# luciddreamer-cvlab/LucidDreamer

Hardware: AMD Instinct MI355X
Metric: views/sec fwd+bwd @1080p (1e6 Gaussians) (higher is better)
Workload: dtype f32

## Files before the change

### luciddreamer_amd/csrc/api.hip

```cpp
#include "common.h"
#include "../../include/lucid_raster.h"
#include "lr_src_hash.h"

#include <cstdio>
#include <cstdlib>
#include <cstddef>
#include <cstring>
#include <cmath>
#include <map>
#include <atomic>
#include <chrono>
#include <mutex>
#include <thread>
#include <string>
#include <vector>

namespace {

thread_local std::string g_last_error;

int fail(int code, const std::string& msg)
{
    g_last_error = msg;
    return code;
// ... 215 lines not shown
        return a.buf;
    }
    if (a.P != P) return nullptr;
    for (int k = 0; k < 5; k++) if (a.tgt[k] != tgt[k]) return nullptr;
    return a.buf;
}

struct RawArgs { const float* sh_rest; const float* opacity_raw; float* dL_dsh_rest; };

static int forward_core(lr_alloc_fn geom_alloc, void* geom_user, lr_alloc_fn binning_alloc, void* binning_user,
               lr_alloc_fn img_alloc, void* img_user, int P, int D, int M, const float* background,
               int width, int height, const float* means3D, const float* shs, const float* colors_precomp,
               const float* opacities, const float* scales, float scale_modifier, const float* rotations,
               const float* cov3D_precomp, const float* viewmatrix, const float* projmatrix,
               const float* cam_pos, float tan_fovx, float tan_fovy, int prefiltered, float* out_color,
               float* out_depth, int* radii, int debug, long long binning_capacity, void* stream_, const RawArgs* raw)
{
    using namespace lr;
    const bool antialiasing = g_antialiasing.load(std::memory_order_relaxed) != 0;
    hipStream_t s = reinterpret_cast<hipStream_t>(stream_);
    const bool early_header = g_early_request;
    g_early_request = false;
    const bool reset_sticky = take_reset_sticky();
    if (P < 0 || width <= 0 || height <= 0) return fail(LR_ERR_INVALID_ARG, "P, width, height must be positive");
    if (!geom_alloc || !binning_alloc || !img_alloc) return fail(LR_ERR_INVALID_ARG, "allocator callbacks are required");
    if (!background || !viewmatrix || !projmatrix || !cam_pos || !out_color || !out_depth)
        return fail(LR_ERR_INVALID_ARG, "background/viewmatrix/projmatrix/cam_pos/out_color/out_depth are required");
    if (P > 0 && (!means3D || !opacities || !radii)) return fail(LR_ERR_INVALID_ARG, "means3D/opacities/radii are required");
    if (P > 0 && shs == nullptr && colors_precomp == nullptr)
        return fail(LR_ERR_INVALID_ARG, "For non-RGB, provide precomputed Gaussian colors!");
    if (P > 0 && cov3D_precomp == nullptr && (scales == nullptr || rotations == nullptr))
        return fail(LR_ERR_INVALID_ARG, "provide scales+rotations or cov3D_precomp");
    if (shs != nullptr && (D < 0 || D > 3 || (D + 1) * (D + 1) > M))
        return fail(LR_ERR_INVALID_ARG, "SH degree must be 0..3 and (D+1)^2 <= M");
    if (binning_capacity < 0 || binning_capacity > 0xFFFFFFF0ll) return fail(LR_ERR_INVALID_ARG, "bad binning_capacity");

    const int gx = (width + TILE_X - 1) / TILE_X, gy = (height + TILE_Y - 1) / TILE_Y;
    const int num_tiles = gx * gy;

    const GeomLayout GL = geom_layout(P);
    const ImgLayout IL = img_layout(width, height);
// ... 110 lines not shown
                                               R_bound, &bp, scratch->words, (uint32_t)n_sum_words, s);
            if (rc == -2) return fail(LR_ERR_INVALID_ARG, "image / instance count too large: tile and slot bits exceed the 64-bit sort word");
            if (rc != 0) return fail(LR_ERR_HIP, "could not reserve LDS for the binning kernels");
            ranges_written = true;
            guard.armed = false;
            LR_DEBUG_SYNC(debug, s, "tile binning");
        }
    } else {
        (void)binning_alloc(bin_layout(0).total, binning_user);
    }
    if (!ranges_written) LR_HIP_CHECK(hipMemsetAsync(ranges, 0, (size_t)num_tiles * sizeof(uint2), s));

    { ProfScope ps(ST_RENDER_FWD, s);
    launch_render_fwd(width, height, gx, gy, ranges, point_list, list_gid, rec, background, final_T, n_contrib, out_color,
                      out_depth, quad_hits, hdr, seg_list, ckpt, reinterpret_cast<uint32_t*>(img + IL.tile_seg0),
                      reinterpret_cast<float4*>(img + IL.c_final), inst_hint, s); }
    LR_DEBUG_SYNC(debug, s, "render");
    LR_HIP_CHECK(hipGetLastError());

    if (binning_capacity == 0 && prefiltered && P > 0) {
        uint32_t trap = 0;
        LR_HIP_CHECK(hipMemcpyAsync(&trap, &hdr->prefilter_trap, 4, hipMemcpyDeviceToHost, s));
        LR_HIP_CHECK(hipStreamSynchronize(s));
        if (trap) return fail(LR_ERR_PREFILTERED, "Point is filtered although prefiltered is set. This shouldn't happen!");
    }
    return num_rendered;
}

int lr_forward(lr_alloc_fn geom_alloc, void* geom_user, lr_alloc_fn binning_alloc, void* binning_user,
               lr_alloc_fn img_alloc, void* img_user, int P, int D, int M, const float* background,
               int width, int height, const float* means3D, const float* shs, const float* colors_precomp,
// ... 403 lines not shown
    unsigned int mask = LR_ACC_MEAN2D | LR_ACC_OPACITY | LR_ACC_MEAN3D;
    if (a->acc_color) mask |= LR_ACC_COLOR;
    if (a->acc_cov3D) mask |= LR_ACC_COV3D;
    if (a->acc_sh) mask |= LR_ACC_SH;
    if (a->acc_scale) mask |= LR_ACC_SCALE;
    if (a->acc_rot) mask |= LR_ACC_ROT;

    lr::ViewsInFlight overlap(n_streams);
    for (int v = 0; v < n_views; v++) {
        const int si = v % n_streams;
        hipStream_t s = g_view_streams[si];
        char* slot = workspace + (size_t)si * SL.total;
        SliceCookie cg = { slot + SL.geom, SL.img - SL.geom }, ci = { slot + SL.img, SL.bin - SL.img },
                    cb = { slot + SL.bin, SL.color - SL.bin };
        float* color = (a->out_color && a->out_color[v]) ? a->out_color[v] : reinterpret_cast<float*>(slot + SL.color);
        float* depth = (a->out_depth && a->out_depth[v]) ? a->out_depth[v] : reinterpret_cast<float*>(slot + SL.depth);
        int* radii = (a->out_radii && a->out_radii[v]) ? a->out_radii[v] : reinterpret_cast<int*>(slot + SL.radii);
        g_reset_sticky = v < n_streams;
        int rc = lr_forward(slice_alloc, &cg, slice_alloc, &cb, slice_alloc, &ci, P, D, M, a->background, width, height,
                            a->means3D, a->shs, a->colors_precomp, a->opacities, a->scales, a->scale_modifier, a->rotations,
                            a->cov3D_precomp, a->viewmatrices[v], a->projmatrices[v], a->cam_positions[v], a->tan_fovx[v],
                            a->tan_fovy[v], 0, color, depth, radii, 0, binning_capacity, s);
        if (rc < 0 && rc != LR_NUM_RENDERED_ON_DEVICE) return rc;
        const float* view_grad = with_loss ? nullptr : a->dL_dpix[v];
        const float* view_depth_grad = a->dL_ddepth ? a->dL_ddepth[v] : nullptr;
        const float* view_alpha_grad = a->dL_dalpha ? a->dL_dalpha[v] : nullptr;
        float* alpha_out = (a->out_alpha && a->out_alpha[v]) ? a->out_alpha[v] : nullptr;
        const float* final_T = reinterpret_cast<const float*>(slot + SL.img + img_layout(width, height).final_T);
        if (alpha_out && !with_mask_loss) launch_render_alpha(final_T, (long long)width * height, alpha_out, s);
        if (with_loss) {
            const float* cmask = with_mask_loss ? masks[v] : nullptr;
            float* gimg = reinterpret_cast<float*>(slot + SL.grad_img);
            float* out_v = a->out_losses + loss_stride * (size_t)v;
            launch_loss_forward(3, height, width, color, targets[v], a->lambda_dssim, out_v, slot + SL.loss_ws, s, true, cmask);
            launch_loss_backward(3, height, width, color, targets[v], a->lambda_dssim, nullptr, slot + SL.loss_ws, gimg, s, out_v,
                                 nullptr, cmask);
            view_grad = gimg;
// ... 597 lines not shown
```

### luciddreamer_amd/csrc/common.h

```cpp
#pragma once
#include <hip/hip_runtime.h>
#include <stdint.h>
#include <stddef.h>

namespace lr {

constexpr int TILE_X = 16;
constexpr int TILE_Y = 16;
constexpr int TILE_PIX = TILE_X * TILE_Y;
constexpr int WAVE = 64;

struct __attribute__((aligned(16))) GaussRec {
    float x, y, ca, cb;
    float cc, opacity, r, g;
    float b, depth, qmax, pad1;
};
static_assert(sizeof(GaussRec) == 48, "GaussRec must be 48 bytes");

struct __attribute__((aligned(16))) GradRec {
    float dmx, dmy, dca, dcb;
    float dcc, dop, dr, dg;
    float db, pad0, pad1, pad2;
};
static_assert(sizeof(GradRec) == 48, "GradRec must be 48 bytes");
// ... 281 lines not shown
enum { TILE_MAP_BANDS = 0, TILE_MAP_PLAIN = 1 };
int blend_tile_map(int num_tiles);
__device__ __forceinline__ int blend_tile(int map, int num_tiles)
{
    int t = (int)blockIdx.x;
    if (map == TILE_MAP_BANDS) {
        const int per = (num_tiles + 7) >> 3;
        t = (int)(blockIdx.x & 7) * per + (int)(blockIdx.x >> 3);
    }
    return t < num_tiles ? t : -1;
}
void launch_render_fwd(int W, int H, int gx, int gy, const uint2* ranges, const uint32_t* point_list,
                       const uint32_t* list_gid, const GaussRec* rec, const float* bg, float* final_T,
                       uint32_t* n_contrib, float* out_color, float* out_depth, uint8_t* quad_hits,
                       GeomHeader* hdr, uint2* seg_list, float4* ckpt, uint32_t* tile_seg0, float4* c_final,
                       long long inst_hint, hipStream_t s);
void launch_render_alpha(const float* final_T, long long n, float* alpha, hipStream_t s);
void launch_render_bwd(int W, int H, int gx, int gy, const uint2* ranges, const uint32_t* point_list,
                       const GaussRec* rec, const float* bg, const float* final_T,
                       const uint32_t* n_contrib, const float* dL_dpix, char* bin_base, const GeomHeader* hdr,
                       const uint32_t* tile_seg0, const float4* c_final, long long seg_bound, hipStream_t s,
                       const float* dL_ddepth = nullptr, const float* depth_img = nullptr, const float* dL_dalpha = nullptr);
__device__ __forceinline__ void adam_one(float gi, float& mi, float& vi, float& pi, float w1, float beta2, float w2,
                                         float bc2_sqrt, float eps, float step_size)
{
    mi = __builtin_fmaf(w1, gi - mi, mi);
    vi = vi * beta2;
    vi = __builtin_fmaf(w2 * gi, gi, vi);
    const float denom = sqrtf(vi) / bc2_sqrt + eps;
    pi = __builtin_fmaf(-step_size, mi / denom, pi);
}
// ... 57 lines not shown
```

### luciddreamer_amd/csrc/preprocess.hip

```cpp
#include <cstddef>
#include "common.h"

namespace lr {

namespace {

__device__ constexpr float SH_C0 = 0.28209479177387814f;
__device__ constexpr float SH_C1 = 0.4886025119029199f;
__device__ constexpr float SH_C2[5] = { 1.0925484305920792f, -1.0925484305920792f, 0.31539156525252005f,
                                        -1.0925484305920792f, 0.5462742152960396f };
__device__ constexpr float SH_C3[7] = { -0.5900435899266435f, 2.890611442640554f, -0.4570457994644658f,
                                        0.3731763325901154f, -0.4570457994644658f, 1.445305721320277f,
                                        -0.5900435899266435f };

struct M3 { float c[3][3]; };

__device__ __forceinline__ M3 m3_mul(const M3& A, const M3& B)
{
    M3 R;
#pragma unroll
    for (int j = 0; j < 3; j++)
#pragma unroll
        for (int i = 0; i < 3; i++)
            R.c[j][i] = A.c[0][i] * B.c[j][0] + A.c[1][i] * B.c[j][1] + A.c[2][i] * B.c[j][2];
// ... 83 lines not shown
    res.x += 0.5f; res.y += 0.5f; res.z += 0.5f;
    clamp_bits = (uint8_t)((res.x < 0 ? 1 : 0) | (res.y < 0 ? 2 : 0) | (res.z < 0 ? 4 : 0));
    res.x = fmaxf(res.x, 0.0f); res.y = fmaxf(res.y, 0.0f); res.z = fmaxf(res.z, 0.0f);
    return res;
}

__device__ __forceinline__ void tile_rect(float px, float py, int radius, int gx, int gy,
                                          int& minx, int& miny, int& maxx, int& maxy)
{
    minx = min(gx, max(0, (int)((px - radius) / TILE_X)));
    miny = min(gy, max(0, (int)((py - radius) / TILE_Y)));
    maxx = min(gx, max(0, (int)((px + radius + TILE_X - 1) / TILE_X)));
    maxy = min(gy, max(0, (int)((py + radius + TILE_Y - 1) / TILE_Y)));
}

constexpr int PP_THREADS = 128;
constexpr int PP_WAVES = PP_THREADS / 64;

template <bool RAW, bool AA>
__global__ void __launch_bounds__(PP_THREADS)
k_preprocess(ViewParams vp, const float* __restrict__ means3D, const float* __restrict__ scales,
             const float* __restrict__ rotations, const float* __restrict__ opacities,
             const float* __restrict__ shs, const float* __restrict__ cov3D_precomp,
             const float* __restrict__ colors_precomp, int prefiltered,
             int* __restrict__ radii, GaussRec* __restrict__ rec, uint8_t* __restrict__ clamped,
             uint32_t* __restrict__ tiles_touched, uint4* __restrict__ hitrec,
             uint32_t* __restrict__ depth_key, GeomHeader* hdr, uint32_t binning_capacity,
             uint32_t* __restrict__ chunk_sums)
{
    __shared__ uint32_t s_list[PP_THREADS];
    __shared__ uint32_t s_wcnt[PP_WAVES];
    const int gid = blockIdx.x * blockDim.x + threadIdx.x;
    uint32_t* const trap = chunk_sums != nullptr ? chunk_sums + 4 * ((size_t)(vp.P + SCAN_TILE - 1) / SCAN_TILE) : &hdr->prefilter_trap;
    const float* __restrict__ V = vp.view;
    const float* __restrict__ Pm = vp.proj;
    {
        const bool in_range = gid < vp.P;
        const size_t li = in_range ? (size_t)gid : 0;
        const float vz1 = V[2] * means3D[3 * li] + V[6] * means3D[3 * li + 1] + V[10] * means3D[3 * li + 2] + V[14];
        const bool pass = in_range && !(vz1 <= 0.2f);
        if (in_range && !pass) {
            if (prefiltered) *trap = 1;
            radii[gid] = 0; tiles_touched[gid] = 0;
            if (depth_key) depth_key[gid] = 0xFFFFFFFFu;
        }
        const uint64_t m = __ballot(pass);
        const int w = threadIdx.x >> 6, l = threadIdx.x & 63;
// ... 12 lines not shown
    const int idx = live ? (int)s_list[threadIdx.x] : 0;

    int radius_out = 0;
    uint32_t tiles_out = 0;
    uint32_t area_ref = 0;
    uint32_t key_out = 0xFFFFFFFFu;

    const size_t li = (size_t)idx;
    const float px_w = means3D[3 * li], py_w = means3D[3 * li + 1], pz_w = means3D[3 * li + 2];
    const float vx = V[0] * px_w + V[4] * py_w + V[8] * pz_w + V[12];
    const float vy = V[1] * px_w + V[5] * py_w + V[9] * pz_w + V[13];
    const float vz = V[2] * px_w + V[6] * py_w + V[10] * pz_w + V[14];

    do {
        if (!live) break;
        const float hx = Pm[0] * px_w + Pm[4] * py_w + Pm[8] * pz_w + Pm[12];
        const float hy = Pm[1] * px_w + Pm[5] * py_w + Pm[9] * pz_w + Pm[13];
        const float hw = Pm[3] * px_w + Pm[7] * py_w + Pm[11] * pz_w + Pm[15];
        const float p_w = 1.0f / (hw + 0.0000001f);
        const float ndcx = hx * p_w, ndcy = hy * p_w;

        float c3[6];
        if (cov3D_precomp != nullptr) {
#pragma unroll
            for (int i = 0; i < 6; i++) c3[i] = cov3D_precomp[6 * (size_t)idx + i];
        } else {
            float sx = scales[3 * (size_t)idx], sy = scales[3 * (size_t)idx + 1], sz = scales[3 * (size_t)idx + 2];
            const float4 q = reinterpret_cast<const float4*>(rotations)[idx];
            float r = q.x, x = q.y, y = q.z, z = q.w;
            if (RAW) {
// ... 236 lines not shown
    __shared__ uint16_t s_near[PL_POOL];
    __shared__ int s_radius[PL_POOL];
    __shared__ uint32_t s_tiles[PL_POOL];
    __shared__ float s_mid[6][PL_POOL];
    __shared__ float s_coef[AA ? PL_POOL : 1];
    __shared__ uint32_t s_mid_id[PL_POOL];
    __shared__ uint32_t s_tests[PL_POOL];
    __shared__ uint2 s_rect[PL_POOL];
    __shared__ uint32_t s_mask[PL_POOL][2];
    __shared__ uint32_t s_wcnt[PL_ROUNDS * PL_WAVES];
    __shared__ uint32_t s_nmid;
    __shared__ uint32_t s_sum[3];
    const int tid = threadIdx.x, w = tid >> 6, l = tid & 63;
    const int base = blockIdx.x * PL_POOL;
    uint32_t* const trap = chunk_sums != nullptr ? chunk_sums + 4 * ((size_t)(vp.P + SCAN_TILE - 1) / SCAN_TILE) : &hdr->prefilter_trap;
    if (tid == 0) { s_nmid = 0u; s_sum[0] = 0u; s_sum[1] = 0u; s_sum[2] = 0u; }
    const float* __restrict__ V = vp.view;

    bool pass[PL_ROUNDS];
    uint64_t m[PL_ROUNDS];
#pragma unroll
    for (int r = 0; r < PL_ROUNDS; r++) {
        const int loc = r * PL_THREADS + tid, gid = base + loc;
        const bool in_range = gid < vp.P;
        const size_t li = in_range ? (size_t)gid : 0;
        const float vz1 = V[2] * means3D[3 * li] + V[6] * means3D[3 * li + 1] + V[10] * means3D[3 * li + 2] + V[14];
        pass[r] = in_range && !(vz1 <= 0.2f);
        if (in_range && !pass[r] && prefiltered) *trap = 1;
        s_radius[loc] = 0; s_tiles[loc] = 0u;
        m[r] = __ballot(pass[r]);
        if (l == 0) s_wcnt[r * PL_WAVES + w] = (uint32_t)__popcll(m[r]);
    }
    lds_barrier();
    uint32_t n_near = 0;
#pragma unroll
    for (int r = 0; r < PL_ROUNDS; r++) {
        uint32_t before = n_near;
#pragma unroll
        for (int i = 0; i < PL_WAVES; i++) { if (i < w) before += s_wcnt[r * PL_WAVES + i]; n_near += s_wcnt[r * PL_WAVES + i]; }
        if (pass[r]) s_near[before + __popcll(m[r] & ((1ull << l) - 1ull))] = (uint16_t)(r * PL_THREADS + tid);
    }
    lds_barrier();

    for (uint32_t i0 = 0; i0 < n_near; i0 += PL_THREADS) {
        const uint32_t i = i0 + (uint32_t)tid;
        Projected pj;
        bool ok = false;
        uint32_t loc = 0;
        if (i < n_near) {
            loc = s_near[i];
            ok = project_gaussian<RAW, AA>(vp, base + (int)loc, means3D, scales, rotations, cov3D_precomp, pj);
        }
        const uint64_t mk = __ballot(ok);
        uint32_t wbase = 0;
        if (l == 0 && mk != 0ull) wbase = atomicAdd(&s_nmid, (uint32_t)__popcll(mk));
        wbase = (uint32_t)__shfl((int)wbase, 0);
        if (ok) {
            const uint32_t slot = wbase + (uint32_t)__popcll(mk & ((1ull << l) - 1ull));
            s_mid[0][slot] = pj.pix; s_mid[1][slot] = pj.piy; s_mid[2][slot] = pj.con_a; s_mid[3][slot] = pj.con_b;
            s_mid[4][slot] = pj.con_c; s_mid[5][slot] = pj.vz;
            if constexpr (AA) s_coef[slot] = pj.coef;
            s_mid_id[slot] = loc; s_radius[loc] = pj.radius;
        }
    }
    lds_barrier();
// ... 151 lines not shown
```

### luciddreamer_amd/csrc/render_fwd.hip

```cpp
#include "common.h"

namespace lr {

namespace {

constexpr int THREADS = 256;
constexpr int NWAVES = THREADS / 64;
constexpr int BATCH = 256;

struct PixState { float T, Cr, Cg, Cb, D, acc; uint32_t last; };

template <bool STRICT>
__device__ __forceinline__ void fwd_pixel(PixState& p, uint64_t& done, const float qA, const float qB, const float qC,
                                          const float r0, const float r1,
                                          const float dx, const float op, const float cr, const float cg, const float cb,
                                          const float depth, const uint32_t pos0)
{
    float power;
    const float alpha = fminf(0.99f, op * gauss_weight<STRICT>(qA, qB, qC, r0, r1, dx, power));
    const float test_T = p.T * (1.0f - alpha);
    const uint64_t pass = ~done & __builtin_amdgcn_ballot_w64(power <= 0.0f) & __builtin_amdgcn_ballot_w64(alpha >= 1.0f / 255.0f);
    const uint64_t low_T = __builtin_amdgcn_ballot_w64(test_T < 0.0001f);
    const uint64_t stop = pass & low_T;
    const bool use = __builtin_amdgcn_inverse_ballot_w64(pass & ~low_T);
    done |= stop;
    const float wgt = use ? alpha * p.T : 0.f;
    p.Cr += cr * wgt; p.Cg += cg * wgt; p.Cb += cb * wgt; p.D += depth * wgt; p.acc += wgt;
    p.T = use ? test_T : p.T;
    if (stop != 0ull) {
        asm volatile("");
        p.last = __builtin_amdgcn_inverse_ballot_w64(stop) ? pos0 : p.last;
    }
}

__device__ __forceinline__ void fwd_step(PixState& p, uint64_t& done, const float alpha, const float power, const uint64_t enable,
                                         const float cr, const float cg, const float cb, const float depth, const uint32_t pos0)
{
    const float test_T = p.T * (1.0f - alpha);
    const uint64_t pass = enable & ~done & __builtin_amdgcn_ballot_w64(power <= 0.0f) & __builtin_amdgcn_ballot_w64(alpha >= 1.0f / 255.0f);
    const uint64_t low_T = __builtin_amdgcn_ballot_w64(test_T < 0.0001f);
    const uint64_t stop = pass & low_T;
    const bool use = __builtin_amdgcn_inverse_ballot_w64(pass & ~low_T);
    done |= stop;
    const float wgt = use ? alpha * p.T : 0.f;
    p.Cr += cr * wgt; p.Cg += cg * wgt; p.Cb += cb * wgt; p.D += depth * wgt; p.acc += wgt;
    p.T = use ? test_T : p.T;
    p.last = __builtin_amdgcn_inverse_ballot_w64(stop) ? pos0 : p.last;
}

constexpr int PAIR_MIN_LIST = 1024;
template <bool STRICT, bool PAIR>
__global__ void __launch_bounds__(THREADS)
k_render_fwd(int W, int H, int gx, int num_tiles, int tile_map, const uint2* __restrict__ ranges,
             const uint32_t* __restrict__ point_list, const uint32_t* __restrict__ list_gid,
             const GaussRec* __restrict__ rec,
             const float* __restrict__ bg, float* __restrict__ final_T, uint32_t* __restrict__ n_contrib,
             float* __restrict__ out_color, float* __restrict__ out_depth, uint8_t* __restrict__ quad_hits,
             GeomHeader* __restrict__ hdr, uint2* __restrict__ seg_list, float4* __restrict__ ckpt,
             uint32_t* __restrict__ tile_seg0, float4* __restrict__ c_final)
{
    __shared__ float4 s_q0[BATCH];
    __shared__ float4 s_q1[BATCH];
    __shared__ float4 s_q2[BATCH];
    __shared__ float2 s_q3[BATCH];
    __shared__ int s_wdone[NWAVES];
    __shared__ uint32_t s_seg0;

    const int tile = blend_tile(tile_map, num_tiles);
    if (tile < 0) return;
    const int tx = tile % gx, ty = tile / gx;
    const int tid = threadIdx.x, w = tid >> 6, l = tid & 63;
    const int x0 = tx * TILE_X + (w & 1) * 8, y0 = ty * TILE_Y + (w >> 1) * 8;
    const int px = x0 + (l & 7), py = y0 + (l >> 3);
    const bool inside = px < W && py < H;
    const float pxf = (float)px, pyf = (float)py;
    const float bx0 = (float)x0, bx1 = (float)(x0 + 7), by0 = (float)y0, by1 = (float)(y0 + 7);

    const uint2 range = ranges[tile];
    const int total = (int)(range.y - range.x);

    PixState A = { 1.0f, 0.f, 0.f, 0.f, 0.f, 0.000001f, 0u };
    uint64_t done = __builtin_amdgcn_ballot_w64(!inside);
    bool wave_done = done == ~0ull;

    static_assert(BATCH == BWD_SEG, "a staging round of the forward is one segment of the backward");
    const int n_seg = total > 0 ? (total - 1) / BWD_SEG : 0;
    uint32_t seg0 = 0;
    int n_ck = 0;
    if (n_seg > 0) {
        if (tid == 0) { s_seg0 = atomicAdd(&hdr->n_seg, (uint32_t)n_seg); tile_seg0[tile] = s_seg0; }
        lds_barrier();
        seg0 = s_seg0;
        for (int g = 1 + tid; g <= n_seg; g += THREADS) seg_list[seg0 + g - 1] = make_uint2((uint32_t)tile, (uint32_t)g);
    }

    for (int base = 0; base < total; base += BATCH) {
// ... 37 lines not shown
                    mask &= mask - 1;
                    const bool two = mask != 0ull;
                    const int k1 = two ? __ffsll((long long)mask) - 1 : k0;
                    mask &= mask - 1;
                    const int j0 = sb + k0, j1 = sb + k1;
                    float4 a0 = s_q0[j0], a1 = s_q0[j1];
                    float4 b0 = s_q1[j0], b1 = s_q1[j1];
                    const float4 c0 = s_q2[j0], c1 = s_q2[j1];
                    asm volatile("" : "+v"(a0.x), "+v"(a0.y), "+v"(a0.z), "+v"(a0.w), "+v"(b0.x), "+v"(a1.x), "+v"(a1.y), "+v"(a1.z), "+v"(a1.w), "+v"(b1.x));
                    float r00, r01, r10, r11, power0, power1;
                    gauss_row<STRICT>(a0.w, b0.x, a0.y - pyf, r00, r01);
                    gauss_row<STRICT>(a1.w, b1.x, a1.y - pyf, r10, r11);
                    float alpha0 = fminf(0.99f, b0.y * gauss_weight<STRICT>(a0.z, a0.w, b0.x, r00, r01, a0.x - pxf, power0));
                    float alpha1 = fminf(0.99f, b1.y * gauss_weight<STRICT>(a1.z, a1.w, b1.x, r10, r11, a1.x - pxf, power1));
                    asm volatile("" : "+v"(alpha0), "+v"(alpha1), "+v"(power0), "+v"(power1));
                    fwd_step(A, done, alpha0, power0, ~0ull, c0.x, c0.y, c0.z, b0.z, (uint32_t)(base + j0));
                    fwd_step(A, done, alpha1, power1, two ? ~0ull : 0ull, c1.x, c1.y, c1.z, b1.z, (uint32_t)(base + j1));
                }
            } else
            while (mask) {
                const int k = __ffsll((long long)mask) - 1;
                mask &= mask - 1;
                const int j = sb + k;
                const float4 a = s_q0[j];
                const float4 b = s_q1[j];
                const float4 c = s_q2[j];
                const uint32_t pos0 = (uint32_t)(base + j);
                const float dy = a.y - pyf;
                float r0, r1;
                gauss_row<STRICT>(a.w, b.x, dy, r0, r1);
                fwd_pixel<STRICT>(A, done, a.z, a.w, b.x, r0, r1, a.x - pxf, b.y, c.x, c.y, c.z, b.z, pos0);
            }
            if (done == ~0ull) { wave_done = true; break; }
        }
    }

    if (inside) {
        const size_t N = (size_t)W * H;
        const size_t pix = (size_t)py * W + px;
        final_T[pix] = A.T;
        n_contrib[pix] = __builtin_amdgcn_inverse_ballot_w64(done) ? A.last : (uint32_t)total;
        const float fr = A.Cr + A.T * bg[0], fg = A.Cg + A.T * bg[1], fb = A.Cb + A.T * bg[2];
        out_color[pix] = fr;
        out_color[N + pix] = fg;
        out_color[2 * N + pix] = fb;
        if (n_seg > 0) c_final[pix] = make_float4(fr, fg, fb, 0.f);
        out_depth[pix] = (A.acc > 0.5f) ? A.D / A.acc : 0.0f;
    }
}



constexpr int TSTAGE = 64;
template <bool STRICT>
__device__ __forceinline__ void
render_fwd_tile(int W, int H, int gx, int num_tiles, int tile_map, const uint2* __restrict__ ranges,
                  const uint32_t* __restrict__ point_list, const uint32_t* __restrict__ list_gid,
                  const GaussRec* __restrict__ rec,
                  const float* __restrict__ bg, float* __restrict__ final_T, uint32_t* __restrict__ n_contrib,
                  float* __restrict__ out_color, float* __restrict__ out_depth, uint8_t* __restrict__ quad_hits,
                  GeomHeader* __restrict__ hdr, uint2* __restrict__ seg_list, float4* __restrict__ ckpt,
                  uint32_t* __restrict__ tile_seg0, float4* __restrict__ c_final)
{
    __shared__ float4 s_q0[TSTAGE];
    __shared__ float4 s_q1[TSTAGE];
    __shared__ float4 s_q2[TSTAGE];

    const int tile = blend_tile(tile_map, num_tiles);
    if (tile < 0) return;
    const int tx = tile % gx, ty = tile / gx;
    const int l = threadIdx.x;
    const int x0 = tx * TILE_X, y0 = ty * TILE_Y;
    const int pxl = x0 + (l & 7), pyt = y0 + (l >> 3);
    const float pxf[2] = { (float)pxl, (float)(pxl + 8) }, pyf[2] = { (float)pyt, (float)(pyt + 8) };

    const uint2 range = ranges[tile];
    const int total = (int)(range.y - range.x);

    PixState A[4];
    uint64_t done[4];
    bool inside[4];
#pragma unroll
    for (int q = 0; q < 4; q++) {
        A[q] = PixState{ 1.0f, 0.f, 0.f, 0.f, 0.f, 0.000001f, 0u };
        inside[q] = pxl + (q & 1) * 8 < W && pyt + (q >> 1) * 8 < H;
        done[q] = __builtin_amdgcn_ballot_w64(!inside[q]);
    }

    static_assert(BWD_SEG % TSTAGE == 0, "checkpoints fall on round boundaries");
    const int n_seg = total > 0 ? (total - 1) / BWD_SEG : 0;
    uint32_t seg0 = 0;
    if (n_seg > 0) {
        if (l == 0) { seg0 = atomicAdd(&hdr->n_seg, (uint32_t)n_seg); tile_seg0[tile] = seg0; }
        seg0 = (uint32_t)__builtin_amdgcn_readfirstlane((int)seg0);
        for (int g = 1 + l; g <= n_seg; g += 64) seg_list[seg0 + g - 1] = make_uint2((uint32_t)tile, (uint32_t)g);
    }

    const uint32_t* __restrict__ lgid = list_gid + range.x;
    uint32_t id_next = total > 0 ? lgid[min(l, total - 1)] : 0u;
// ... 38 lines not shown
            mask &= mask - 1;
            const float4 fa = s_q0[k];
            const float4 fb = s_q1[k];
            const float4 fc = s_q2[k];
            const uint32_t pos0 = (uint32_t)(base + k);
            const uint64_t bit = 1ull << k;
#pragma unroll
            for (int row = 0; row < 2; row++) {
                if (((m[2 * row] | m[2 * row + 1]) & bit) == 0ull) continue;
                float r0, r1;
                gauss_row<STRICT>(fa.w, fb.x, fa.y - pyf[row], r0, r1);
#pragma unroll
                for (int col = 0; col < 2; col++) {
                    const int q = 2 * row + col;
                    if ((m[q] & bit) == 0ull) continue;
                    fwd_pixel<STRICT>(A[q], done[q], fa.z, fa.w, fb.x, r0, r1, fa.x - pxf[col], fb.y, fc.x, fc.y, fc.z, fb.z, pos0);
                    if (done[q] == ~0ull) {
                        m[q] = 0ull;
                        mask &= (m[0] | m[1]) | (m[2] | m[3]);
                    }
                }
            }
        }
    }

    const size_t N = (size_t)W * H;
#pragma unroll
    for (int q = 0; q < 4; q++) {
        if (!inside[q]) continue;
        const int px = pxl + (q & 1) * 8, py = pyt + (q >> 1) * 8;
        const size_t pix = (size_t)py * W + px;
        final_T[pix] = A[q].T;
        n_contrib[pix] = __builtin_amdgcn_inverse_ballot_w64(done[q]) ? A[q].last : (uint32_t)total;
        const float fr = A[q].Cr + A[q].T * bg[0], fg = A[q].Cg + A[q].T * bg[1], fb = A[q].Cb + A[q].T * bg[2];
        out_color[pix] = fr;
        out_color[N + pix] = fg;
        out_color[2 * N + pix] = fb;
        if (n_seg > 0) c_final[pix] = make_float4(fr, fg, fb, 0.f);
        out_depth[pix] = (A[q].acc > 0.5f) ? A[q].D / A[q].acc : 0.0f;
    }
}
#define LR_FWD_TILE_PARAMS int W, int H, int gx, int num_tiles, int tile_map, const uint2* __restrict__ ranges,                 \
                  const uint32_t* __restrict__ point_list, const uint32_t* __restrict__ list_gid,                              \
                  const GaussRec* __restrict__ rec,                                                                            \
                  const float* __restrict__ bg, float* __restrict__ final_T, uint32_t* __restrict__ n_contrib,                 \
                  float* __restrict__ out_color, float* __restrict__ out_depth, uint8_t* __restrict__ quad_hits,               \
                  GeomHeader* __restrict__ hdr, uint2* __restrict__ seg_list, float4* __restrict__ ckpt,                       \
                  uint32_t* __restrict__ tile_seg0, float4* __restrict__ c_final
#define LR_FWD_TILE_PASS W, H, gx, num_tiles, tile_map, ranges, point_list, list_gid, rec, bg, final_T, n_contrib, out_color,  \
                  out_depth, quad_hits, hdr, seg_list, ckpt, tile_seg0, c_final
template <bool STRICT>
__global__ void __launch_bounds__(64) __attribute__((amdgpu_waves_per_eu(8, 8), amdgpu_num_vgpr(64)))
k_render_fwd_tile(LR_FWD_TILE_PARAMS)
{
    render_fwd_tile<STRICT>(LR_FWD_TILE_PASS);
}

}

void launch_render_fwd(int W, int H, int gx, int gy, const uint2* ranges, const uint32_t* point_list,
                       const uint32_t* list_gid, const GaussRec* rec, const float* bg, float* final_T,
                       uint32_t* n_contrib, float* out_color, float* out_depth, uint8_t* quad_hits,
                       GeomHeader* hdr, uint2* seg_list, float4* ckpt, uint32_t* tile_seg0, float4* c_final,
                       long long inst_hint, hipStream_t s)
{
    const int num_tiles = gx * gy;
    if (num_tiles <= 0) return;
    const int tile_map = blend_tile_map(num_tiles);
    const int grid = ((num_tiles + 7) / 8) * 8;
    const int knob = tune_get(TUNE_FWD_PAIR);
    const bool long_lists = inst_hint > (long long)BATCH * num_tiles;
    const bool tile_shape = knob >= 0 ? knob == 2 : (num_tiles > 3072 && views_in_flight() >= 2 && !long_lists);
#ifdef LR_DIAGNOSTICS
    const bool pair = knob == 1;
#else
    constexpr bool pair = false;
#endif
    const bool strict = tune_get(TUNE_STRICT) > 0;
    note_fwd_shape(tile_shape ? 2 : pair ? 1 : 0);
#define LR_FWD_ARGS W, H, gx, num_tiles, tile_map, ranges, point_list, list_gid, rec, bg, final_T, n_contrib, out_color, out_depth, \
                    quad_hits, hdr, seg_list, ckpt, tile_seg0, c_final
    if (tile_shape) {
        if (strict) hipLaunchKernelGGL((k_render_fwd_tile<true>), dim3(grid), dim3(64), 0, s, LR_FWD_ARGS);
        else hipLaunchKernelGGL((k_render_fwd_tile<false>), dim3(grid), dim3(64), 0, s, LR_FWD_ARGS);
        return;
    }
#define LR_FWD(S, PR) hipLaunchKernelGGL((k_render_fwd<S, PR>), dim3(grid), dim3(THREADS), 0, s, LR_FWD_ARGS)
#ifdef LR_DIAGNOSTICS
    if (pair) { if (strict) LR_FWD(true, true); else LR_FWD(false, true); return; }
#endif
    if (strict) LR_FWD(true, false); else LR_FWD(false, false);
#undef LR_FWD_ARGS
#undef LR_FWD
}

__global__ void __launch_bounds__(256) k_render_alpha(const float* __restrict__ final_T, long long n, float* __restrict__ alpha)
{
    const long long i = (long long)blockIdx.x * 256 + threadIdx.x;
    if (i < n) alpha[i] = 1.0f - final_T[i];
}
__global__ void __launch_bounds__(256) k_render_alpha4(const float4* __restrict__ final_T, long long n4, float4* __restrict__ alpha)
{
    const long long i = (long long)blockIdx.x * 256 + threadIdx.x;
    if (i < n4) {
        const float4 t = final_T[i];
        alpha[i] = make_float4(1.0f - t.x, 1.0f - t.y, 1.0f - t.z, 1.0f - t.w);
// ... 21 lines not shown
```

Baseline: 5955.

## Skip depth accumulation when unused and add cheap off-screen cull in preprocessing

Adds a DEPTH_OUT template path to the forward render kernels. When no consumer of depth exists in the batched fwd+bwd loop, the depth and weight accumulators and the depth store are dropped, which lowers register and store pressure. Also adds a conservative screen-space rejection test, using a bound on the view-space covariance radius, that runs before full projection in both preprocess kernels. Near-list entries are compacted after this test so off-screen Gaussians skip the expensive projection. The risks are a more complex compaction step with extra barriers, and the cull bound must stay conservative or it would drop visible Gaussians.

```diff
diff --git a/luciddreamer_amd/csrc/api.hip b/luciddreamer_amd/csrc/api.hip
--- a/luciddreamer_amd/csrc/api.hip
+++ b/luciddreamer_amd/csrc/api.hip
@@ -253,7 +253,8 @@
                const float* opacities, const float* scales, float scale_modifier, const float* rotations,
                const float* cov3D_precomp, const float* viewmatrix, const float* projmatrix,
                const float* cam_pos, float tan_fovx, float tan_fovy, int prefiltered, float* out_color,
-               float* out_depth, int* radii, int debug, long long binning_capacity, void* stream_, const RawArgs* raw)
+               float* out_depth, int* radii, int debug, long long binning_capacity, void* stream_, const RawArgs* raw,
+               bool depth_out = true)
 {
     using namespace lr;
     const bool antialiasing = g_antialiasing.load(std::memory_order_relaxed) != 0;
@@ -263,7 +264,7 @@
     const bool reset_sticky = take_reset_sticky();
     if (P < 0 || width <= 0 || height <= 0) return fail(LR_ERR_INVALID_ARG, "P, width, height must be positive");
     if (!geom_alloc || !binning_alloc || !img_alloc) return fail(LR_ERR_INVALID_ARG, "allocator callbacks are required");
-    if (!background || !viewmatrix || !projmatrix || !cam_pos || !out_color || !out_depth)
+    if (!background || !viewmatrix || !projmatrix || !cam_pos || !out_color || (depth_out && !out_depth))
         return fail(LR_ERR_INVALID_ARG, "background/viewmatrix/projmatrix/cam_pos/out_color/out_depth are required");
     if (P > 0 && (!means3D || !opacities || !radii)) return fail(LR_ERR_INVALID_ARG, "means3D/opacities/radii are required");
     if (P > 0 && shs == nullptr && colors_precomp == nullptr)
@@ -404,7 +405,7 @@
     { ProfScope ps(ST_RENDER_FWD, s);
     launch_render_fwd(width, height, gx, gy, ranges, point_list, list_gid, rec, background, final_T, n_contrib, out_color,
                       out_depth, quad_hits, hdr, seg_list, ckpt, reinterpret_cast<uint32_t*>(img + IL.tile_seg0),
-                      reinterpret_cast<float4*>(img + IL.c_final), inst_hint, s); }
+                      reinterpret_cast<float4*>(img + IL.c_final), inst_hint, s, depth_out); }
     LR_DEBUG_SYNC(debug, s, "render");
     LR_HIP_CHECK(hipGetLastError());
 
@@ -838,13 +839,15 @@
         SliceCookie cg = { slot + SL.geom, SL.img - SL.geom }, ci = { slot + SL.img, SL.bin - SL.img },
                     cb = { slot + SL.bin, SL.color - SL.bin };
         float* color = (a->out_color && a->out_color[v]) ? a->out_color[v] : reinterpret_cast<float*>(slot + SL.color);
-        float* depth = (a->out_depth && a->out_depth[v]) ? a->out_depth[v] : reinterpret_cast<float*>(slot + SL.depth);
+        const bool depth_reader = (a->out_depth && a->out_depth[v]) || (a->dL_ddepth && a->dL_ddepth[v]) || with_depth_loss;
+        float* depth = (a->out_depth && a->out_depth[v]) ? a->out_depth[v]
+                       : depth_reader ? reinterpret_cast<float*>(slot + SL.depth) : nullptr;
         int* radii = (a->out_radii && a->out_radii[v]) ? a->out_radii[v] : reinterpret_cast<int*>(slot + SL.radii);
         g_reset_sticky = v < n_streams;
-        int rc = lr_forward(slice_alloc, &cg, slice_alloc, &cb, slice_alloc, &ci, P, D, M, a->background, width, height,
-                            a->means3D, a->shs, a->colors_precomp, a->opacities, a->scales, a->scale_modifier, a->rotations,
-                            a->cov3D_precomp, a->viewmatrices[v], a->projmatrices[v], a->cam_positions[v], a->tan_fovx[v],
-                            a->tan_fovy[v], 0, color, depth, radii, 0, binning_capacity, s);
+        int rc = forward_core(slice_alloc, &cg, slice_alloc, &cb, slice_alloc, &ci, P, D, M, a->background, width, height,
+                              a->means3D, a->shs, a->colors_precomp, a->opacities, a->scales, a->scale_modifier, a->rotations,
+                              a->cov3D_precomp, a->viewmatrices[v], a->projmatrices[v], a->cam_positions[v], a->tan_fovx[v],
+                              a->tan_fovy[v], 0, color, depth, radii, 0, binning_capacity, s, nullptr, depth_reader);
         if (rc < 0 && rc != LR_NUM_RENDERED_ON_DEVICE) return rc;
         const float* view_grad = with_loss ? nullptr : a->dL_dpix[v];
         const float* view_depth_grad = a->dL_ddepth ? a->dL_ddepth[v] : nullptr;
diff --git a/luciddreamer_amd/csrc/common.h b/luciddreamer_amd/csrc/common.h
--- a/luciddreamer_amd/csrc/common.h
+++ b/luciddreamer_amd/csrc/common.h
@@ -319,7 +319,7 @@
                        const uint32_t* list_gid, const GaussRec* rec, const float* bg, float* final_T,
                        uint32_t* n_contrib, float* out_color, float* out_depth, uint8_t* quad_hits,
                        GeomHeader* hdr, uint2* seg_list, float4* ckpt, uint32_t* tile_seg0, float4* c_final,
-                       long long inst_hint, hipStream_t s);
+                       long long inst_hint, hipStream_t s, bool depth_out = true);
 void launch_render_alpha(const float* final_T, long long n, float* alpha, hipStream_t s);
 void launch_render_bwd(int W, int H, int gx, int gy, const uint2* ranges, const uint32_t* point_list,
                        const GaussRec* rec, const float* bg, const float* final_T,
diff --git a/luciddreamer_amd/csrc/preprocess.hip b/luciddreamer_amd/csrc/preprocess.hip
--- a/luciddreamer_amd/csrc/preprocess.hip
+++ b/luciddreamer_amd/csrc/preprocess.hip
@@ -121,6 +121,75 @@
     maxy = min(gy, max(0, (int)((py + radius + TILE_Y - 1) / TILE_Y)));
 }
 
+struct RejectView { float kw, gw, gh; };
+
+__device__ __forceinline__ RejectView reject_view(const ViewParams& vp)
+{
+    const float* __restrict__ V = vp.view;
+    float g[3][3];
+#pragma unroll
+    for (int i = 0; i < 3; i++)
+#pragma unroll
+        for (int j = 0; j < 3; j++)
+            g[i][j] = V[4 * i] * V[4 * j] + V[4 * i + 1] * V[4 * j + 1] + V[4 * i + 2] * V[4 * j + 2];
+    const float r0 = fabsf(g[0][0]) + fabsf(g[0][1]) + fabsf(g[0][2]);
+    const float r1 = fabsf(g[1][0]) + fabsf(g[1][1]) + fabsf(g[1][2]);
+    const float r2 = fabsf(g[2][0]) + fabsf(g[2][1]) + fabsf(g[2][2]);
+    const float wn = fmaxf(fmaxf(r0, r1), r2) + (r0 + r1 + r2) * 0.0f;
+    const float limx = 1.3f * vp.tan_fovx, limy = 1.3f * vp.tan_fovy;
+    const float K = vp.focal_x * vp.focal_x * (1.0f + limx * limx) + vp.focal_y * vp.focal_y * (1.0f + limy * limy);
+    float kw = K * wn;
+    if (!(kw >= 0x1p-40f && kw <= 0x1p40f)) kw = __builtin_inff();
+    RejectView rv = { kw, (float)(vp.gx * TILE_X), (float)(vp.gy * TILE_Y) };
+    return rv;
+}
+
+template <bool RAW>
+__device__ __forceinline__ bool screen_reject(const ViewParams& vp, const RejectView& rv, int idx,
+                                              const float* __restrict__ means3D, const float* __restrict__ scales,
+                                              const float* __restrict__ rotations, const float* __restrict__ cov3D_precomp)
+{
+    const float* __restrict__ V = vp.view;
+    const float* __restrict__ Pm = vp.proj;
+    const size_t li = (size_t)idx;
+    const float px_w = means3D[3 * li], py_w = means3D[3 * li + 1], pz_w = means3D[3 * li + 2];
+    const float vz = V[2] * px_w + V[6] * py_w + V[10] * pz_w + V[14];
+    const float hx = Pm[0] * px_w + Pm[4] * py_w + Pm[8] * pz_w + Pm[12];
+    const float hy = Pm[1] * px_w + Pm[5] * py_w + Pm[9] * pz_w + Pm[13];
+    const float hw = Pm[3] * px_w + Pm[7] * py_w + Pm[11] * pz_w + Pm[15];
+    const float p_w = __builtin_amdgcn_rcpf(hw + 0.0000001f);
+    const float pix = ((hx * p_w + 1.0f) * (float)vp.W - 1.0f) * 0.5f;
+    const float piy = ((hy * p_w + 1.0f) * (float)vp.H - 1.0f) * 0.5f;
+
+    float lam3, rho = 1.0f;
+    if (cov3D_precomp != nullptr) {
+        const float* c = cov3D_precomp + 6 * li;
+        const float dg = c[0] * c[0] + c[3] * c[3] + c[5] * c[5], od = c[1] * c[1] + c[2] * c[2] + c[4] * c[4];
+        lam3 = __builtin_amdgcn_sqrtf(dg + 2.0f * od) * (1.0f + 0x1p-20f);
+    } else {
+        float sx = scales[3 * li], sy = scales[3 * li + 1], sz = scales[3 * li + 2];
+        const float4 q = reinterpret_cast<const float4*>(rotations)[idx];
+        float r = q.x, x = q.y, y = q.z, z = q.w;
+        if (RAW) {
+            sx = act_scale(sx); sy = act_scale(sy); sz = act_scale(sz);
+            const float inv = act_quat_inv_norm(r, x, y, z);
+            r *= inv; x *= inv; y *= inv; z *= inv;
+        }
+        const float guard = (sx + sy + sz) * 0.0f;
+        const float sm = vp.scale_modifier * fmaxf(fmaxf(fabsf(sx), fabsf(sy)), fabsf(sz));
+        const float v2 = x * x + y * y + z * z;
+        rho = 1.0f + 4.0f * v2 * ((r * r + v2) - 1.0f);
+        rho = rho < 1.0f ? 1.0f : rho;
+        lam3 = sm * sm * rho + guard;
+    }
+    const float inv_z = __builtin_amdgcn_rcpf(vz);
+    const float B = rv.kw * ((inv_z * inv_z) * lam3);
+    const float R = (3.0f * (1.0f + 0x1p-10f)) * __builtin_amdgcn_sqrtf(B + 0.62f) + 2.0f;
+    const float mx = R + 0x1p-10f * (fabsf(pix) + rv.gw), my = R + 0x1p-10f * (fabsf(piy) + rv.gh);
+    const bool off = (pix + mx < 0.0f) || (pix - mx > rv.gw) || (piy + my < 0.0f) || (piy - my > rv.gh);
+    return off && vz <= 0x1p50f && rho <= 0x1p40f;
+}
+
 constexpr int PP_THREADS = 128;
 constexpr int PP_WAVES = PP_THREADS / 64;
 
@@ -137,7 +206,9 @@
 {
     __shared__ uint32_t s_list[PP_THREADS];
     __shared__ uint32_t s_wcnt[PP_WAVES];
+    __shared__ RejectView s_rej;
     const int gid = blockIdx.x * blockDim.x + threadIdx.x;
+    if (threadIdx.x == 0) s_rej = reject_view(vp);
     uint32_t* const trap = chunk_sums != nullptr ? chunk_sums + 4 * ((size_t)(vp.P + SCAN_TILE - 1) / SCAN_TILE) : &hdr->prefilter_trap;
     const float* __restrict__ V = vp.view;
     const float* __restrict__ Pm = vp.proj;
@@ -180,6 +251,7 @@
 
     do {
         if (!live) break;
+        if (screen_reject<RAW>(vp, s_rej, idx, means3D, scales, rotations, cov3D_precomp)) break;
         const float hx = Pm[0] * px_w + Pm[4] * py_w + Pm[8] * pz_w + Pm[12];
         const float hy = Pm[1] * px_w + Pm[5] * py_w + Pm[9] * pz_w + Pm[13];
         const float hw = Pm[3] * px_w + Pm[7] * py_w + Pm[11] * pz_w + Pm[15];
@@ -446,7 +518,8 @@
     const int tid = threadIdx.x, w = tid >> 6, l = tid & 63;
     const int base = blockIdx.x * PL_POOL;
     uint32_t* const trap = chunk_sums != nullptr ? chunk_sums + 4 * ((size_t)(vp.P + SCAN_TILE - 1) / SCAN_TILE) : &hdr->prefilter_trap;
-    if (tid == 0) { s_nmid = 0u; s_sum[0] = 0u; s_sum[1] = 0u; s_sum[2] = 0u; }
+    __shared__ RejectView s_rej;
+    if (tid == 0) { s_nmid = 0u; s_sum[0] = 0u; s_sum[1] = 0u; s_sum[2] = 0u; s_rej = reject_view(vp); }
     const float* __restrict__ V = vp.view;
 
     bool pass[PL_ROUNDS];
@@ -474,13 +547,42 @@
     }
     lds_barrier();
 
+    uint32_t* const s_keep = s_tests;
+    {
+        const RejectView rv = s_rej;
+        uint32_t kloc[PL_ROUNDS];
+#pragma unroll
+        for (int r = 0; r < PL_ROUNDS; r++) {
+            const uint32_t i = (uint32_t)(r * PL_THREADS + tid);
+            pass[r] = false;
+            kloc[r] = 0u;
+            if (i < n_near) {
+                kloc[r] = s_near[i];
+                pass[r] = !screen_reject<RAW>(vp, rv, base + (int)kloc[r], means3D, scales, rotations, cov3D_precomp);
+            }
+            m[r] = __ballot(pass[r]);
+            if (l == 0) s_wcnt[r * PL_WAVES + w] = (uint32_t)__popcll(m[r]);
+        }
+        lds_barrier();
+        uint32_t n_keep = 0;
+#pragma unroll
+        for (int r = 0; r < PL_ROUNDS; r++) {
+            uint32_t before = n_keep;
+#pragma unroll
+            for (int i = 0; i < PL_WAVES; i++) { if (i < w) before += s_wcnt[r * PL_WAVES + i]; n_keep += s_wcnt[r * PL_WAVES + i]; }
+            if (pass[r]) s_keep[before + __popcll(m[r] & ((1ull << l) - 1ull))] = kloc[r];
+        }
+        lds_barrier();
+        n_near = n_keep;
+    }
+
     for (uint32_t i0 = 0; i0 < n_near; i0 += PL_THREADS) {
         const uint32_t i = i0 + (uint32_t)tid;
         Projected pj;
         bool ok = false;
         uint32_t loc = 0;
         if (i < n_near) {
-            loc = s_near[i];
+            loc = s_keep[i];
             ok = project_gaussian<RAW, AA>(vp, base + (int)loc, means3D, scales, rotations, cov3D_precomp, pj);
         }
         const uint64_t mk = __ballot(ok);
diff --git a/luciddreamer_amd/csrc/render_fwd.hip b/luciddreamer_amd/csrc/render_fwd.hip
--- a/luciddreamer_amd/csrc/render_fwd.hip
+++ b/luciddreamer_amd/csrc/render_fwd.hip
@@ -8,10 +8,15 @@
 constexpr int NWAVES = THREADS / 64;
 constexpr int BATCH = 256;
 
-struct PixState { float T, Cr, Cg, Cb, D, acc; uint32_t last; };
-
-template <bool STRICT>
-__device__ __forceinline__ void fwd_pixel(PixState& p, uint64_t& done, const float qA, const float qB, const float qC,
+template <bool DEPTH_OUT> struct PixState;
+template <> struct PixState<true> { float T, Cr, Cg, Cb, D, acc; uint32_t last; };
+template <> struct PixState<false> { float T, Cr, Cg, Cb; uint32_t last; };
+template <bool DEPTH_OUT> __device__ __forceinline__ PixState<DEPTH_OUT> pix_state_init();
+template <> __device__ __forceinline__ PixState<true> pix_state_init<true>() { return PixState<true>{ 1.0f, 0.f, 0.f, 0.f, 0.f, 0.000001f, 0u }; }
+template <> __device__ __forceinline__ PixState<false> pix_state_init<false>() { return PixState<false>{ 1.0f, 0.f, 0.f, 0.f, 0u }; }
+
+template <bool STRICT, bool DEPTH_OUT>
+__device__ __forceinline__ void fwd_pixel(PixState<DEPTH_OUT>& p, uint64_t& done, const float qA, const float qB, const float qC,
                                           const float r0, const float r1,
                                           const float dx, const float op, const float cr, const float cg, const float cb,
                                           const float depth, const uint32_t pos0)
@@ -25,7 +30,8 @@
     const bool use = __builtin_amdgcn_inverse_ballot_w64(pass & ~low_T);
     done |= stop;
     const float wgt = use ? alpha * p.T : 0.f;
-    p.Cr += cr * wgt; p.Cg += cg * wgt; p.Cb += cb * wgt; p.D += depth * wgt; p.acc += wgt;
+    p.Cr += cr * wgt; p.Cg += cg * wgt; p.Cb += cb * wgt;
+    if constexpr (DEPTH_OUT) { p.D += depth * wgt; p.acc += wgt; }
     p.T = use ? test_T : p.T;
     if (stop != 0ull) {
         asm volatile("");
@@ -33,7 +39,8 @@
     }
 }
 
-__device__ __forceinline__ void fwd_step(PixState& p, uint64_t& done, const float alpha, const float power, const uint64_t enable,
+template <bool DEPTH_OUT>
+__device__ __forceinline__ void fwd_step(PixState<DEPTH_OUT>& p, uint64_t& done, const float alpha, const float power, const uint64_t enable,
                                          const float cr, const float cg, const float cb, const float depth, const uint32_t pos0)
 {
     const float test_T = p.T * (1.0f - alpha);
@@ -43,13 +50,14 @@
     const bool use = __builtin_amdgcn_inverse_ballot_w64(pass & ~low_T);
     done |= stop;
     const float wgt = use ? alpha * p.T : 0.f;
-    p.Cr += cr * wgt; p.Cg += cg * wgt; p.Cb += cb * wgt; p.D += depth * wgt; p.acc += wgt;
+    p.Cr += cr * wgt; p.Cg += cg * wgt; p.Cb += cb * wgt;
+    if constexpr (DEPTH_OUT) { p.D += depth * wgt; p.acc += wgt; }
     p.T = use ? test_T : p.T;
     p.last = __builtin_amdgcn_inverse_ballot_w64(stop) ? pos0 : p.last;
 }
 
 constexpr int PAIR_MIN_LIST = 1024;
-template <bool STRICT, bool PAIR>
+template <bool STRICT, bool PAIR, bool DEPTH_OUT>
 __global__ void __launch_bounds__(THREADS)
 k_render_fwd(int W, int H, int gx, int num_tiles, int tile_map, const uint2* __restrict__ ranges,
              const uint32_t* __restrict__ point_list, const uint32_t* __restrict__ list_gid,
@@ -79,7 +87,7 @@
     const uint2 range = ranges[tile];
     const int total = (int)(range.y - range.x);
 
-    PixState A = { 1.0f, 0.f, 0.f, 0.f, 0.f, 0.000001f, 0u };
+    PixState<DEPTH_OUT> A = pix_state_init<DEPTH_OUT>();
     uint64_t done = __builtin_amdgcn_ballot_w64(!inside);
     bool wave_done = done == ~0ull;
 
@@ -147,8 +155,8 @@
                     float alpha0 = fminf(0.99f, b0.y * gauss_weight<STRICT>(a0.z, a0.w, b0.x, r00, r01, a0.x - pxf, power0));
                     float alpha1 = fminf(0.99f, b1.y * gauss_weight<STRICT>(a1.z, a1.w, b1.x, r10, r11, a1.x - pxf, power1));
                     asm volatile("" : "+v"(alpha0), "+v"(alpha1), "+v"(power0), "+v"(power1));
-                    fwd_step(A, done, alpha0, power0, ~0ull, c0.x, c0.y, c0.z, b0.z, (uint32_t)(base + j0));
-                    fwd_step(A, done, alpha1, power1, two ? ~0ull : 0ull, c1.x, c1.y, c1.z, b1.z, (uint32_t)(base + j1));
+                    fwd_step<DEPTH_OUT>(A, done, alpha0, power0, ~0ull, c0.x, c0.y, c0.z, b0.z, (uint32_t)(base + j0));
+                    fwd_step<DEPTH_OUT>(A, done, alpha1, power1, two ? ~0ull : 0ull, c1.x, c1.y, c1.z, b1.z, (uint32_t)(base + j1));
                 }
             } else
             while (mask) {
@@ -162,7 +170,7 @@
                 const float dy = a.y - pyf;
                 float r0, r1;
                 gauss_row<STRICT>(a.w, b.x, dy, r0, r1);
-                fwd_pixel<STRICT>(A, done, a.z, a.w, b.x, r0, r1, a.x - pxf, b.y, c.x, c.y, c.z, b.z, pos0);
+                fwd_pixel<STRICT, DEPTH_OUT>(A, done, a.z, a.w, b.x, r0, r1, a.x - pxf, b.y, c.x, c.y, c.z, b.z, pos0);
             }
             if (done == ~0ull) { wave_done = true; break; }
         }
@@ -178,14 +186,14 @@
         out_color[N + pix] = fg;
         out_color[2 * N + pix] = fb;
         if (n_seg > 0) c_final[pix] = make_float4(fr, fg, fb, 0.f);
-        out_depth[pix] = (A.acc > 0.5f) ? A.D / A.acc : 0.0f;
+        if constexpr (DEPTH_OUT) out_depth[pix] = (A.acc > 0.5f) ? A.D / A.acc : 0.0f;
     }
 }
 
 
 
 constexpr int TSTAGE = 64;
-template <bool STRICT>
+template <bool STRICT, bool DEPTH_OUT>
 __device__ __forceinline__ void
 render_fwd_tile(int W, int H, int gx, int num_tiles, int tile_map, const uint2* __restrict__ ranges,
                   const uint32_t* __restrict__ point_list, const uint32_t* __restrict__ list_gid,
@@ -210,12 +218,12 @@
     const uint2 range = ranges[tile];
     const int total = (int)(range.y - range.x);
 
-    PixState A[4];
+    PixState<DEPTH_OUT> A[4];
     uint64_t done[4];
     bool inside[4];
 #pragma unroll
     for (int q = 0; q < 4; q++) {
-        A[q] = PixState{ 1.0f, 0.f, 0.f, 0.f, 0.f, 0.000001f, 0u };
+        A[q] = pix_state_init<DEPTH_OUT>();
         inside[q] = pxl + (q & 1) * 8 < W && pyt + (q >> 1) * 8 < H;
         done[q] = __builtin_amdgcn_ballot_w64(!inside[q]);
     }
@@ -284,7 +292,7 @@
                 for (int col = 0; col < 2; col++) {
                     const int q = 2 * row + col;
                     if ((m[q] & bit) == 0ull) continue;
-                    fwd_pixel<STRICT>(A[q], done[q], fa.z, fa.w, fb.x, r0, r1, fa.x - pxf[col], fb.y, fc.x, fc.y, fc.z, fb.z, pos0);
+                    fwd_pixel<STRICT, DEPTH_OUT>(A[q], done[q], fa.z, fa.w, fb.x, r0, r1, fa.x - pxf[col], fb.y, fc.x, fc.y, fc.z, fb.z, pos0);
                     if (done[q] == ~0ull) {
                         m[q] = 0ull;
                         mask &= (m[0] | m[1]) | (m[2] | m[3]);
@@ -307,7 +315,7 @@
         out_color[N + pix] = fg;
         out_color[2 * N + pix] = fb;
         if (n_seg > 0) c_final[pix] = make_float4(fr, fg, fb, 0.f);
-        out_depth[pix] = (A[q].acc > 0.5f) ? A[q].D / A[q].acc : 0.0f;
+        if constexpr (DEPTH_OUT) out_depth[pix] = (A[q].acc > 0.5f) ? A[q].D / A[q].acc : 0.0f;
     }
 }
 #define LR_FWD_TILE_PARAMS int W, int H, int gx, int num_tiles, int tile_map, const uint2* __restrict__ ranges,                 \
@@ -319,11 +327,11 @@
                   uint32_t* __restrict__ tile_seg0, float4* __restrict__ c_final
 #define LR_FWD_TILE_PASS W, H, gx, num_tiles, tile_map, ranges, point_list, list_gid, rec, bg, final_T, n_contrib, out_color,  \
                   out_depth, quad_hits, hdr, seg_list, ckpt, tile_seg0, c_final
-template <bool STRICT>
+template <bool STRICT, bool DEPTH_OUT>
 __global__ void __launch_bounds__(64) __attribute__((amdgpu_waves_per_eu(8, 8), amdgpu_num_vgpr(64)))
 k_render_fwd_tile(LR_FWD_TILE_PARAMS)
 {
-    render_fwd_tile<STRICT>(LR_FWD_TILE_PASS);
+    render_fwd_tile<STRICT, DEPTH_OUT>(LR_FWD_TILE_PASS);
 }
 
 }
@@ -332,7 +340,7 @@
                        const uint32_t* list_gid, const GaussRec* rec, const float* bg, float* final_T,
                        uint32_t* n_contrib, float* out_color, float* out_depth, uint8_t* quad_hits,
                        GeomHeader* hdr, uint2* seg_list, float4* ckpt, uint32_t* tile_seg0, float4* c_final,
-                       long long inst_hint, hipStream_t s)
+                       long long inst_hint, hipStream_t s, bool depth_out)
 {
     const int num_tiles = gx * gy;
     if (num_tiles <= 0) return;
@@ -342,7 +350,7 @@
     const bool long_lists = inst_hint > (long long)BATCH * num_tiles;
     const bool tile_shape = knob >= 0 ? knob == 2 : (num_tiles > 3072 && views_in_flight() >= 2 && !long_lists);
 #ifdef LR_DIAGNOSTICS
-    const bool pair = knob == 1;
+    const bool pair = knob == 1 && depth_out;
 #else
     constexpr bool pair = false;
 #endif
@@ -351,15 +359,18 @@
 #define LR_FWD_ARGS W, H, gx, num_tiles, tile_map, ranges, point_list, list_gid, rec, bg, final_T, n_contrib, out_color, out_depth, \
                     quad_hits, hdr, seg_list, ckpt, tile_seg0, c_final
     if (tile_shape) {
-        if (strict) hipLaunchKernelGGL((k_render_fwd_tile<true>), dim3(grid), dim3(64), 0, s, LR_FWD_ARGS);
-        else hipLaunchKernelGGL((k_render_fwd_tile<false>), dim3(grid), dim3(64), 0, s, LR_FWD_ARGS);
+#define LR_FWD_TILE(S, DO) hipLaunchKernelGGL((k_render_fwd_tile<S, DO>), dim3(grid), dim3(64), 0, s, LR_FWD_ARGS)
+        if (depth_out) { if (strict) LR_FWD_TILE(true, true); else LR_FWD_TILE(false, true); }
+        else { if (strict) LR_FWD_TILE(true, false); else LR_FWD_TILE(false, false); }
+#undef LR_FWD_TILE
         return;
     }
-#define LR_FWD(S, PR) hipLaunchKernelGGL((k_render_fwd<S, PR>), dim3(grid), dim3(THREADS), 0, s, LR_FWD_ARGS)
+#define LR_FWD(S, PR, DO) hipLaunchKernelGGL((k_render_fwd<S, PR, DO>), dim3(grid), dim3(THREADS), 0, s, LR_FWD_ARGS)
 #ifdef LR_DIAGNOSTICS
-    if (pair) { if (strict) LR_FWD(true, true); else LR_FWD(false, true); return; }
+    if (pair) { if (strict) LR_FWD(true, true, true); else LR_FWD(false, true, true); return; }
 #endif
-    if (strict) LR_FWD(true, false); else LR_FWD(false, false);
+    if (depth_out) { if (strict) LR_FWD(true, false, true); else LR_FWD(false, false, true); }
+    else { if (strict) LR_FWD(true, false, false); else LR_FWD(false, false, false); }
 #undef LR_FWD_ARGS
 #undef LR_FWD
 }
```

Result: no change. 6012 (median of 6 runs) (+1.0%).
